# MohamedAbou-Taleb/Iterative-Linear-Quadratic-Regulator

Hardware: AMD Instinct MI355X
Metric: iLQR iterations/sec (batch=4096, T=200, n=4 m=1); backward-pass HBM GB/s (higher is better)
Workload: dtype f32; 1 GPU; c3: under-actuated double pendulum swing-up (run_iLQR_UA_MPC.py params), n=4 m=1 N=200 rk4, batch 4096 trajectories per GPU, 10 parallel line-search alphas per pass covering the 10 reference trials, fixed iterations; batch_per_gpu=4096, horizon=200, n_alpha=10, n_trials=10

## Files before the change

### iterative-linear-quadratic-regulator_amd/csrc/backward_fused16.hpp

```cpp
#pragma once

namespace ilqr {

template <typename T, int TPW, bool PK> struct FusedCfg;
template <> struct FusedCfg<float, 16, false> { static constexpr int P = 8, RU = 8; };
#ifndef ILQR_PK_RU
#define ILQR_PK_RU 5
#endif
#ifndef ILQR_PK_PAD
#define ILQR_PK_PAD 0
#endif
template <> struct FusedCfg<float, 16, true> { static constexpr int P = 4, RU = ILQR_PK_RU; };
template <> struct FusedCfg<double, 16, false> { static constexpr int P = 4, RU = 4; };
template <> struct FusedCfg<float, 4, false> { static constexpr int P = 3, RU = 4; };
template <> struct FusedCfg<double, 4, false> { static constexpr int P = 3, RU = 3; };

template <int NU> constexpr int fused_tl() { return NU == 2 ? 68 : 52; }
template <bool PK, int NU> constexpr int fused_unit_scalars() { return (PK ? 128 : 64) * fused_tl<NU>() + (PK ? 64 * ILQR_PK_PAD : 0); }
template <typename T, int TPW, bool PK, int NU> constexpr int fused_ru() { return (PK && NU == 2 && FusedCfg<T, TPW, PK>::RU > 4) ? 4 : FusedCfg<T, TPW, PK>::RU; }
template <typename T, int TPW, bool PK, int NU = 1> constexpr int fused_lds_bytes() {
    return fused_ru<T, TPW, PK, NU>() * fused_unit_scalars<PK, NU>() * (int)sizeof(T) + (fused_ru<T, TPW, PK, NU>() + 4 + 32 + 4) * 4;
}
static_assert(fused_lds_bytes<float, 16, true, 1>() <= 160 * 1024 && fused_lds_bytes<float, 16, true, 2>() <= 160 * 1024 &&
              fused_lds_bytes<float, 16, false, 2>() <= 160 * 1024 && fused_lds_bytes<double, 16, false, 2>() <= 160 * 1024, "LDS ring exceeds a CU");
template <typename T, int TPW, bool PK> constexpr int fused_threads() { return 64 * (TPW / 4 + FusedCfg<T, TPW, PK>::P); }

template <typename T, int NU> struct FusedStep;
template <> struct FusedStep<float, 1> {
    using Tile = TileQ;
    static ILQR_DEV void load(Tile& t, const float* tp, int i, int j, int l16) {
        const float4 s = *reinterpret_cast<const float4*>(tp + 4 * j);
        const float4 v = *reinterpret_cast<const float4*>(tp + 32 + 4 * j);
        t.skj[0] = s.x; t.skj[1] = s.y; t.skj[2] = s.z; t.skj[3] = s.w;
        t.vj[0] = v.x; t.vj[1] = v.y; t.vj[2] = v.z; t.vj[3] = v.w;
        t.a = tp[l16];
        t.lxx = tp[16 + l16];
        t.c = tp[32 + l16];
    }
    static ILQR_DEV void step(const Tile& c, const LaneConst<float>& lc, int i, int j, float& V, float& vx, float& out, bool& pd) {
        RawTileQ none;
        const i32x4 srd = {0, 0, 0, 0};
        const TileOffsets off = {0, 0, 0};
        float Kj, kff;
        tile16_step_f32<false>(c, lc, V, vx, Kj, kff, pd, none, srd, off, 0);
        out = (i == 0) ? Kj : kff;
    }
    static ILQR_DEV void step_box(const Tile& c, const LaneConst<float>& lc, int i, int j, float u, float lo, float hi,
                                  float& V, float& vx, float& out, bool& pd) {
        RawTileQ none;
        const i32x4 srd = {0, 0, 0, 0};
        const TileOffsets off = {0, 0, 0};
        float Kj, kff;
        tile16_step_f32<false, true>(c, lc, V, vx, Kj, kff, pd, none, srd, off, 0, u, lo, hi);
        out = (i == 0) ? Kj : kff;
    }
};
template <> struct FusedStep<double, 1> {
    using Tile = Tile16<double>;
    static ILQR_DEV void load(Tile& t, const double* tp, int i, int j, int l16) { tile16_load_lds(t, tp, i, j, l16); }
    static ILQR_DEV void step(const Tile& c, const LaneConst<double>& lc, int i, int j, double& V, double& vx, double& out, bool& pd) {
        double Kj, kff;
        tile16_step<double, false>(c, lc, 0.0, V, vx, Kj, kff, pd);
        out = (i == 0) ? Kj : kff;
    }
    static ILQR_DEV void step_box(const Tile& c, const LaneConst<double>& lc, int i, int j, double u, double lo, double hi,
                                  double& V, double& vx, double& out, bool& pd) {
        double Kj, kff;
        tile16_step<double, false, true>(c, lc, 0.0, V, vx, Kj, kff, pd, u, lo, hi);
        out = (i == 0) ? Kj : kff;
    }
};
template <> struct FusedStep<float, 2> {
    using Tile = TileQ2;
    static ILQR_DEV void load(Tile& t, const float* tp, int i, int j, int l16) { tileq2_load_lds(t, tp, i, j, l16); }
    static ILQR_DEV void step(const Tile& c, const LaneConst<float>& lc, int i, int j, float& V, float& vx, float& out, bool& pd) {
        const GainSel sel = GainSel::of(i, j);
        tile16m2_step_f32(c, lc, sel, V, vx, out, pd);
    }
};
template <typename T> struct FusedStep<T, 2> {
    using Tile = Tile16M2<T>;
    using V4 = typename Vec4<T>::type;
    static ILQR_DEV void load(Tile& t, const T* tp, int i, int j, int l16) {
        const V4 si = *reinterpret_cast<const V4*>(tp + 4 * i);
        const V4 sj = *reinterpret_cast<const V4*>(tp + 4 * j);
        const V4 g0 = *reinterpret_cast<const V4*>(tp + 32 + 8 * j);
        const V4 g1 = *reinterpret_cast<const V4*>(tp + 36 + 8 * j);
        t.ski[0] = si.x; t.ski[1] = si.y; t.ski[2] = si.z; t.ski[3] = si.w;
        t.skj[0] = sj.x; t.skj[1] = sj.y; t.skj[2] = sj.z; t.skj[3] = sj.w;
        t.gj[0] = g0.x; t.gj[1] = g0.y; t.gj[2] = g0.z; t.gj[3] = g0.w;
        t.gj[4] = g1.x; t.gj[5] = g1.y; t.gj[6] = g1.z; t.gj[7] = g1.w;
        const T* gi = tp + 32 + 8 * i;
        t.gi[0] = gi[0]; t.gi[1] = gi[1]; t.gi[3] = gi[3]; t.gi[4] = gi[4];
        t.lxx = tp[16 + l16];
    }
    static ILQR_DEV void step(const Tile& c, const LaneConst<T>& lc, int i, int j, T& V, T& vx, T& out, bool& pd) {
        T K0, K1, k0, k1;
        tile16m2_step<T, false>(c, lc.m0, lc.m1, T(0), V, vx, K0, K1, k0, k1, pd);
        out = (i == 0) ? K0 : ((i == 1) ? K1 : ((j == 0) ? k0 : k1));
    }
};

ILQR_DEV void compiler_fence() { asm volatile("" ::: "memory"); }
ILQR_DEV int lds_peek(const int* p) { return __hip_atomic_load(p, __ATOMIC_RELAXED, __HIP_MEMORY_SCOPE_WORKGROUP); }
ILQR_DEV void lds_poke(int* p, int v) { __hip_atomic_store(p, v, __ATOMIC_RELAXED, __HIP_MEMORY_SCOPE_WORKGROUP); }

template <typename T, typename Dyn, int INTEG, int TPW, bool PK, bool BOX, bool HET> struct FusedRoles {
    static constexpr int NX = Dyn::NX, NU = Dyn::NU;
    static_assert(!BOX || (NU == 1 && fused_tl<1>() > kTile16), "control limits: n_u = 1, u_t in the tile's padding");
    static_assert((NU == 1 && NX >= 2 && NX <= 4) || (NX == 4 && NU == 2), "the fused sweep serves the DPP tiles: n_u = 1, or (4, 2)");
    static_assert(TPW == 16 || TPW == 4, "16 or 4 trajectories per workgroup");
    static_assert(!PK || (sizeof(T) == 4 && TPW == 16 && INTEG != ILQR_INT_BACKWARD_EULER), "pair producers: fp32, 16-trajectory workgroups, explicit integrators");
    using Cfg = FusedCfg<T, TPW, PK>;
    static constexpr int P = Cfg::P, RU = fused_ru<T, TPW, PK, NU>(), TL = fused_tl<NU>();
    static constexpr int NV = (NU == 2 ? kTile16M2 : kTile16) / 4;
    static constexpr int NSW = TPW / 4;
    static constexpr int UT = PK ? 128 : 64;
    static constexpr int US = UT / TPW;
    static constexpr int UNIT = fused_unit_scalars<PK, NU>();
    static constexpr int PS = 2 * TL + ILQR_PK_PAD;
    static constexpr int R = gain_record(NX, NU);
    using PL = ParamLayout<Dyn::NSYS, NX, NU>;
    using V4 = typename Vec4<T>::type;
    static ILQR_DEV constexpr int tile_off(int r, int tl) { return PK ? ((r / 2) * TPW + tl) * PS + (r % 2) * TL : (r * TPW + tl) * TL; }
    static ILQR_DEV constexpr int step_off(int r) { return PK ? (r / 2) * TPW * PS + (r % 2) * TL : r * TPW * TL; }

    struct Lds {
        T* ring;
        int* ready;
        int* done;
        int* s_slot;
        int* s_stat;
    };
    static ILQR_DEV Lds carve(unsigned char* base) {
        Lds L;
        L.ring = reinterpret_cast<T*>(base);
        L.ready = reinterpret_cast<int*>(base + (size_t)RU * UNIT * sizeof(T));
        L.done = L.ready + RU;
        L.s_slot = L.done + 4;
        L.s_stat = L.s_slot + 16;
        return L;
    }

    static ILQR_DEV void head(const KArgs<T>& a, const Lds& L, int b0, int lane, bool do_select, bool count) {
        bool still = false;
        if (lane < 16) {
            const int b = b0 + lane;
            int slot = 0, st = -1;
            if (lane < TPW && b < a.B) {
                if (do_select) {
                    still = select_candidates(a, b, true, slot, st);
                } else {
                    st = a.status[b];
                    slot = a.cur_slot[b];
                }
                a.cur_slot[b] = traj_active(st) ? 0 : slot;
            }
            L.s_slot[lane] = slot;
            L.s_stat[lane] = st;
        } else if (lane < 16 + RU + 4) {
            L.ready[lane - 16] = 0;
        }
        if (do_select && count) {
            const unsigned long long m = __ballot(still);
            if (lane == 0 && m) atomicAdd(&a.counters[a.counter_idx], (int)__popcll(m));
            if (blockIdx.x == 0 && lane == 0) a.counters[(a.counter_idx + 1) % kCounterRing] = 0;
        }
    }
    static ILQR_DEV bool any_active(const Lds& L) {
        bool any = false;
#pragma unroll
        for (int q = 0; q < 16; ++q) any = any || traj_active(L.s_stat[q]);
        return any;
    }

    static ILQR_DEV void sweep(const KArgs<T>& a, const Lds& L, int b0, int wave, int lane, ClockProbe& cp) {
        const size_t B = a.B;
        const int N = a.N;
        const int tid = threadIdx.x;
        (void)tid;
        __builtin_amdgcn_s_setprio(2);
        const int l16 = lane & 15, i = l16 >> 2, j = l16 & 3;
        const int tl = 4 * wave + (lane >> 4);
        const int gidx = b0 + tl;
        const bool valid = gidx < a.B;
        const int b = valid ? gidx : a.B - 1;
        const int st = L.s_stat[tl];
        const bool act = valid && traj_active(st);
        const int slot = act ? L.s_slot[tl] : 0;
        T ph[HET ? PL::TOTAL : 1];
        if constexpr (HET) {
#pragma unroll
            for (int q = 0; q < PL::TOTAL; ++q) ph[q] = a.params[q];
            load_row<PL::Q>(ph, a.rows, B, b);
        }
        const T* __restrict__ pp = HET ? ph : a.params;
        T xN[NX];
        vec_load<T, NX>(a.X + vec_at(B, N + 1, NX, slot, N, b), xN);
        if (act && slot != 0 && l16 == 0) vec_store<T, NX>(a.X + vec_at(B, N + 1, NX, 0, N, b), xN);
        T V = T(0), vx = T(0);
        {
            T g[NX], H[NX][NX];
            Cost<T, Dyn>::l_f_x(pp, xN, g);
            Cost<T, Dyn>::l_f_xx(pp, xN, H);
#pragma unroll
            for (int ii = 0; ii < NX; ++ii) {
// ... 254 lines not shown
```

### iterative-linear-quadratic-regulator_amd/csrc/backward_tile16.hpp

```cpp
#pragma once
#include <type_traits>
#include <utility>

#include "dynamics.hpp"

namespace ilqr {

constexpr int dpp_quad(int a, int b, int c, int d) { return a | (b << 2) | (c << 4) | (d << 6); }
constexpr int kRowRor = 0x120;
constexpr int kDown1 = kRowRor + 12;
constexpr int kDown2 = kRowRor + 8;
constexpr int kDown3 = kRowRor + 4;
constexpr int kRight1 = dpp_quad(1, 2, 3, 0);
constexpr int kRight2 = dpp_quad(2, 3, 0, 1);
constexpr int kRight3 = dpp_quad(3, 0, 1, 2);
constexpr int kSwap1 = dpp_quad(1, 0, 3, 2);

template <int CTRL, int BANK = 0xf, bool BOUND = true> ILQR_DEV int dpp_bits(int old, int v) {
    return __builtin_amdgcn_update_dpp(old, v, CTRL, 0xf, BANK, BOUND);
}
template <int CTRL> ILQR_DEV float dpp(float v) {
    return __int_as_float(dpp_bits<CTRL>(0, __float_as_int(v)));
}
template <int CTRL> ILQR_DEV double dpp(double v) {
// ... 224 lines not shown
    float a, lxx, c;
    ILQR_DEV void issue_first(const i32x4& srd, const TileOffsets& o, int soff) {
        asm volatile(
            "s_nop 4\n\t"
            "buffer_load_dwordx4 %0, %5, %7, %8 offen" ILQR_TILE_NT "\n\t"
            "buffer_load_dwordx4 %1, %5, %7, %8 offen offset:128" ILQR_TILE_NT "\n\t"
            "buffer_load_dword %2, %6, %7, %8 offen" ILQR_TILE_NT "\n\t"
            "buffer_load_dword %3, %6, %7, %8 offen offset:64" ILQR_TILE_NT "\n\t"
            "buffer_load_dword %4, %6, %7, %8 offen offset:128" ILQR_TILE_NT
            : "=&v"(skj), "=&v"(vj), "=&v"(a), "=&v"(lxx), "=&v"(c)
            : "v"(o.vj), "v"(o.vl), "s"(srd), "s"(soff)
            : "memory");
    }
#define ILQR_RAWTILE_PART(NOP, dst, voff, IMM)                                                               \
    asm volatile(NOP "buffer_load_dword" IMM ILQR_TILE_NT : "+&v"(dst) : "v"(voff), "s"(srd), "s"(soff) : "memory")
    template <int K> ILQR_DEV void issue_part(const i32x4& srd, const TileOffsets& o, int soff) {
        if constexpr (K == 0) ILQR_RAWTILE_PART("s_nop 4\n\t", skj, o.vj, "x4 %0, %1, %2, %3 offen");
        if constexpr (K == 1) ILQR_RAWTILE_PART("", vj, o.vj, "x4 %0, %1, %2, %3 offen offset:128");
        if constexpr (K == 2) ILQR_RAWTILE_PART("", a, o.vl, " %0, %1, %2, %3 offen");
        if constexpr (K == 3) ILQR_RAWTILE_PART("", lxx, o.vl, " %0, %1, %2, %3 offen offset:64");
        if constexpr (K == 4) ILQR_RAWTILE_PART("", c, o.vl, " %0, %1, %2, %3 offen offset:128");
    }
    template <int N> ILQR_DEV void wait() {
        asm volatile("s_waitcnt vmcnt(%5)" : "+v"(skj), "+v"(vj), "+v"(a), "+v"(lxx), "+v"(c) : "i"(N) : "memory");
    }
    ILQR_DEV void unpack(TileQ& t) const {
        t.skj[0] = skj.x; t.skj[1] = skj.y; t.skj[2] = skj.z; t.skj[3] = skj.w;
        t.vj[0] = vj.x; t.vj[1] = vj.y; t.vj[2] = vj.z; t.vj[3] = vj.w;
        t.a = a; t.lxx = lxx; t.c = c;
    }
};

#define ILQR_FMAC_DPP_(NOP, acc, w, coef, CTRL)                                                        \
    asm volatile(NOP "v_fmac_f32_dpp %0, %1, %2 " CTRL " row_mask:0xf bank_mask:0xf bound_ctrl:1"        \
                 : "+v"(acc)                                                                           \
                 : "v"(w), "v"(coef))
#define ILQR_FMAC_DPP_FIRST(acc, w, coef, CTRL) ILQR_FMAC_DPP_("s_nop 1\n\t", acc, w, coef, CTRL)
#define ILQR_FMAC_DPP_NEXT(acc, w, coef, CTRL) ILQR_FMAC_DPP_("", acc, w, coef, CTRL)

ILQR_DEV float contract_row(const float* skj, float w, float init) {
    float acc = fmaf(skj[0], w, init);
    ILQR_FMAC_DPP_FIRST(acc, w, skj[1], "quad_perm:[1,2,3,0]");
    ILQR_FMAC_DPP_NEXT(acc, w, skj[2], "quad_perm:[2,3,0,1]");
    ILQR_FMAC_DPP_NEXT(acc, w, skj[3], "quad_perm:[3,0,1,2]");
    return acc;
}
ILQR_DEV double contract_row(const double* skj, double w, double init) {
    double acc = fma(skj[0], w, init);
    acc += skj[1] * dpp<kRight1>(w);
    acc += skj[2] * dpp<kRight2>(w);
    acc += skj[3] * dpp<kRight3>(w);
    return acc;
}
ILQR_DEV float contract_col(const float* ski, float w) {
    float acc = ski[0] * w;
    ILQR_FMAC_DPP_FIRST(acc, w, ski[1], "row_ror:12");
    ILQR_FMAC_DPP_NEXT(acc, w, ski[2], "row_ror:8");
    ILQR_FMAC_DPP_NEXT(acc, w, ski[3], "row_ror:4");
    return acc;
}
ILQR_DEV double contract_col(const double* ski, double w) {
    double acc = ski[0] * w;
    acc += ski[1] * dpp<kDown1>(w);
    acc += ski[2] * dpp<kDown2>(w);
    acc += ski[3] * dpp<kDown3>(w);
    return acc;
}
template <typename T> ILQR_DEV T quad_sum(T v) {
    v += dpp<kSwap1>(v);
    v += dpp<kRight2>(v);
    return v;
}

ILQR_DEV float lane_transpose(float v, int src_byte) {
    return __int_as_float(__builtin_amdgcn_ds_bpermute(src_byte, __float_as_int(v)));
}
ILQR_DEV double lane_transpose(double v, int src_byte) {
    const int lo = __builtin_amdgcn_ds_bpermute(src_byte, __double2loint(v));
    const int hi = __builtin_amdgcn_ds_bpermute(src_byte, __double2hiint(v));
    return __hiloint2double(hi, lo);
}

ILQR_DEV void contract_row2(const float* skj, float w0, float w1, float c0, float c1, float& o0, float& o1) {
    float a0 = fmaf(skj[0], w0, c0), a1 = fmaf(skj[0], w1, c1);
    ILQR_FMAC_DPP_FIRST(a0, w0, skj[1], "quad_perm:[1,2,3,0]");
    ILQR_FMAC_DPP_NEXT(a1, w1, skj[1], "quad_perm:[1,2,3,0]");
    ILQR_FMAC_DPP_NEXT(a0, w0, skj[2], "quad_perm:[2,3,0,1]");
    ILQR_FMAC_DPP_NEXT(a1, w1, skj[2], "quad_perm:[2,3,0,1]");
    ILQR_FMAC_DPP_NEXT(a0, w0, skj[3], "quad_perm:[3,0,1,2]");
    ILQR_FMAC_DPP_NEXT(a1, w1, skj[3], "quad_perm:[3,0,1,2]");
    o0 = a0; o1 = a1;
}
ILQR_DEV void contract_row2(const double* skj, double w0, double w1, double c0, double c1, double& o0, double& o1) {
    o0 = contract_row(skj, w0, c0);
    o1 = contract_row(skj, w1, c1);
}

template <typename T> struct LaneConst {
    T m0, m1;
    int tr_byte;
};

template <typename T, bool REG, bool BOX = false>
ILQR_DEV void tile16_step(const Tile16<T>& c, const LaneConst<T>& lc, T mu, T& V, T& vx, T& Kj, T& kff, bool& pd,
                          T ut = T(0), T blo = T(0), T bhi = T(0)) {
    static_assert(!(BOX && REG), "control limits take the fused kernels, which run without regularisation");
    const T P = contract_col(c.ski, V);
    T pu = c.bi * V;
    pu += dpp<kDown2>(pu);
    pu += dpp<kDown1>(pu);
    T Qux, Qx;
    contract_row2(c.skj, pu, vx, c.vj[2], c.vj[1], Qux, Qx);
    const T Quu = quad_sum(lc.m1 * c.vj[3] + pu * c.vj[0]);
    const T Qu = quad_sum(lc.m0 * c.vj[3] + c.vj[0] * vx);
    const T Qr = REG ? Quu + mu : Quu;
    pd = Qr > T(0);
    const T inv = fast_rcp(Qr);
    Kj = -(Qux * inv);
    kff = -(Qu * inv);
    T Quxi = Qux;
    Quxi = dpp_row<dpp_quad(0, 0, 0, 0), 0x1>(Quxi, Qux);
    Quxi = dpp_row<dpp_quad(1, 1, 1, 1), 0x2>(Quxi, Qux);
    Quxi = dpp_row<dpp_quad(2, 2, 2, 2), 0x4>(Quxi, Qux);
    Quxi = dpp_row<dpp_quad(3, 3, 3, 3), 0x8>(Quxi, Qux);
    const T Qxx = contract_row(c.skj, P, c.lxx);
    if constexpr (!REG) {
        V = Qxx + Quxi * Kj;
        vx = Qx + Kj * Qu;
        if constexpr (BOX) {
            const T lo = blo - ut, hi = bhi - ut;
            const bool out = kff < lo || kff > hi;
            const T kc = clamp_keep_nan(kff, lo, hi);
            const T vxc = Qx + Qux * kc;
            V = out ? Qxx : V;
            vx = out ? vxc : vx;
            Kj = out ? T(0) : Kj;
            kff = kc;
        }
    } else {
        const T Ki = -(Quxi * inv);
        V = Qxx + Ki * (Quu * Kj) + Ki * Qux + Quxi * Kj;
        vx = Qx + Kj * (Quu * kff + Qu) + Qux * kff;
    }
}

#define ILQR_QP1 "quad_perm:[1,2,3,0]"
#define ILQR_QP2 "quad_perm:[2,3,0,1]"
#define ILQR_QP3 "quad_perm:[3,0,1,2]"
#define ILQR_QSW "quad_perm:[1,0,3,2]"
#define ILQR_QB0 "quad_perm:[0,0,0,0]"
#define ILQR_QB1 "quad_perm:[1,1,1,1]"
#define ILQR_QB2 "quad_perm:[2,2,2,2]"
#define ILQR_QB3 "quad_perm:[3,3,3,3]"
template <bool REFILL, bool BOX = false>
ILQR_DEV void tile16_step_f32(const TileQ& c, const LaneConst<float>& lc, float& V, float& vx, float& Kj, float& kff,
                              bool& pd, RawTileQ& prev, const i32x4& srd, const TileOffsets& off, int soff,
                              float ut = 0.0f, float blo = 0.0f, float bhi = 0.0f) {
    using T = float;
    float P, pu, qx, qu, quu, Qxx, Qux, Quxi, t, t2, inv, si1, si2, si3;
#define DPPT " row_mask:0xf bank_mask:0xf bound_ctrl:1\n\t"
#define DPPE " row_mask:0xf bank_mask:0xf bound_ctrl:1"
    asm volatile(
        "v_mov_b32_dpp %[si1], %[a] " ILQR_QB1 DPPT
        "v_mov_b32_dpp %[si2], %[a] " ILQR_QB2 DPPT
        "v_mov_b32_dpp %[si3], %[a] " ILQR_QB3 DPPT
        "v_mul_f32_dpp %[P], %[a], %[V] " ILQR_QB0 DPPT
        "v_mul_f32_dpp %[pu], %[c], %[V] " ILQR_QB0 DPPT
        "v_fma_f32 %[qx], %[sj0], %[vx], %[vj1]\n\t"
        "v_fmac_f32_dpp %[P], %[V], %[si1] row_ror:12" DPPT
        "v_add_f32_dpp %[t], %[pu], %[pu] row_ror:8" DPPE
        : [P] "=&v"(P), [pu] "=&v"(pu), [qx] "=&v"(qx), [t] "=&v"(t), [si1] "=&v"(si1), [si2] "=&v"(si2), [si3] "=&v"(si3)
        : [V] "v"(V), [vx] "v"(vx), [a] "v"(c.a), [c] "v"(c.c), [sj0] "v"(c.skj[0]), [vj1] "v"(c.vj[1]));
    if constexpr (REFILL) prev.template issue_part<0>(srd, off, soff);
    asm volatile(
        "v_fmac_f32_dpp %[qx], %[vx], %[sj1] " ILQR_QP1 DPPT
        "v_fmac_f32_dpp %[P], %[V], %[si2] row_ror:8" DPPT
        "v_add_f32_dpp %[pu], %[t], %[t] row_ror:12" DPPT
        "v_mul_f32 %[qu], %[vj0], %[vx]\n\t"
        "v_fmac_f32_dpp %[qx], %[vx], %[sj2] " ILQR_QP2 DPPT
        "v_fmac_f32_dpp %[P], %[V], %[si3] row_ror:4" DPPE
        : [qx] "+v"(qx), [P] "+v"(P), [qu] "=&v"(qu), [pu] "=&v"(pu)
        : [V] "v"(V), [vx] "v"(vx), [si2] "v"(si2), [si3] "v"(si3), [sj1] "v"(c.skj[1]), [sj2] "v"(c.skj[2]),
          [vj0] "v"(c.vj[0]), [t] "v"(t));
    if constexpr (REFILL) prev.template issue_part<1>(srd, off, soff);
    asm volatile(
        "v_mul_f32 %[quu], %[pu], %[vj0]\n\t"
        "v_fma_f32 %[Qux], %[sj0], %[pu], %[vj2]\n\t"
        "v_fmac_f32_dpp %[qx], %[vx], %[sj3] " ILQR_QP3 DPPT
        "v_fmac_f32 %[quu], %[m1], %[vj3]\n\t"
        "v_fmac_f32 %[qu], %[m0], %[vj3]\n\t"
        "v_fma_f32 %[Qxx], %[sj0], %[P], %[lxx]"
        : [quu] "=&v"(quu), [Qux] "=&v"(Qux), [Qxx] "=&v"(Qxx), [qx] "+v"(qx), [qu] "+v"(qu)
        : [vx] "v"(vx), [sj0] "v"(c.skj[0]), [sj3] "v"(c.skj[3]), [vj0] "v"(c.vj[0]), [vj2] "v"(c.vj[2]),
          [vj3] "v"(c.vj[3]), [lxx] "v"(c.lxx), [m0] "v"(lc.m0), [m1] "v"(lc.m1), [pu] "v"(pu), [P] "v"(P));
    if constexpr (REFILL) prev.template issue_part<2>(srd, off, soff);
    asm volatile(
        "v_fmac_f32_dpp %[Qux], %[pu], %[sj1] " ILQR_QP1 DPPT
        "v_add_f32_dpp %[t2], %[quu], %[quu] " ILQR_QSW DPPT
        "v_add_f32_dpp %[t], %[qu], %[qu] " ILQR_QSW DPPT
        "v_fmac_f32_dpp %[Qxx], %[P], %[sj1] " ILQR_QP1 DPPT
        "v_add_f32_dpp %[quu], %[t2], %[t2] " ILQR_QP2 DPPT
        "v_fmac_f32_dpp %[Qux], %[pu], %[sj2] " ILQR_QP2 DPPE
        : [Qux] "+v"(Qux), [Qxx] "+v"(Qxx), [quu] "+v"(quu), [t] "=&v"(t), [t2] "=&v"(t2)
        : [sj1] "v"(c.skj[1]), [sj2] "v"(c.skj[2]), [pu] "v"(pu), [P] "v"(P), [qu] "v"(qu));
    if constexpr (REFILL) prev.template issue_part<3>(srd, off, soff);
    asm volatile(
        "v_add_f32_dpp %[qu], %[t], %[t] " ILQR_QP2 DPPT
        "v_rcp_f32 %[inv], %[quu]\n\t"
        "v_fmac_f32_dpp %[Qxx], %[P], %[sj2] " ILQR_QP2 DPPT
        "v_fmac_f32_dpp %[Qux], %[pu], %[sj3] " ILQR_QP3 DPPT
        "v_fma_f32 %[e], -%[quu], %[inv], 1.0\n\t"
        "v_fmac_f32_dpp %[Qxx], %[P], %[sj3] " ILQR_QP3 DPPT
        "v_mov_b32_dpp %[Quxi], %[Qux] " ILQR_QB0 " row_mask:0xf bank_mask:0x1\n\t"
        "v_fmac_f32 %[inv], %[e], %[inv]\n\t"
        "v_mov_b32_dpp %[Quxi], %[Qux] " ILQR_QB1 " row_mask:0xf bank_mask:0x2\n\t"
        "v_mov_b32_dpp %[Quxi], %[Qux] " ILQR_QB2 " row_mask:0xf bank_mask:0x4\n\t"
        "v_mov_b32_dpp %[Quxi], %[Qux] " ILQR_QB3 " row_mask:0xf bank_mask:0x8"
        : [Quxi] "=&v"(Quxi), [Qxx] "+v"(Qxx), [Qux] "+v"(Qux), [qu] "=&v"(qu), [inv] "=&v"(inv), [e] "=&v"(t2)
        : [sj2] "v"(c.skj[2]), [sj3] "v"(c.skj[3]), [pu] "v"(pu), [P] "v"(P), [t] "v"(t), [quu] "v"(quu));
    if constexpr (REFILL) prev.template issue_part<4>(srd, off, soff);
#undef DPPT
#undef DPPE
    pd = quu > 0.0f;
    Kj = -(Qux * inv);
    kff = -(qu * inv);
    V = fmaf(Quxi, Kj, Qxx);
    vx = fmaf(Kj, qu, qx);
    if constexpr (BOX) {
        const T lo = blo - ut, hi = bhi - ut;
        const bool out = kff < lo || kff > hi;
        const T kc = clamp_keep_nan(kff, lo, hi);
        const T vxc = fmaf(Qux, kc, qx);
        V = out ? Qxx : V;
        vx = out ? vxc : vx;
        Kj = out ? T(0) : Kj;
        kff = kc;
    }
}

constexpr int kTile16PinLds = 84 * 1024;

template <typename T, bool REG, int NXA>
__global__ void __launch_bounds__(256) backward_tile16_kernel(KArgs<T> a) {
#ifndef ILQR_TILE16_D32
#define ILQR_TILE16_D32 10
#endif
    constexpr bool SPREAD = sizeof(T) == 4 && !REG;
    constexpr int D = SPREAD ? ILQR_TILE16_D32 : sizeof(T) == 4 ? 10 : 7;
    constexpr int R = gain_record(NXA, 1);
    const int lane = threadIdx.x & 63;
    const int l16 = lane & 15, i = l16 >> 2, j = l16 & 3;
    const int gidx = (blockIdx.x * 4 + (threadIdx.x >> 6)) * 4 + (lane >> 4);
    const bool valid = gidx < a.B;
    const int b = valid ? gidx : a.B - 1;
    const int st = a.status[b];
    const bool act = valid && traj_active(st);
    if (__ballot(act) == 0ull) return;
    if (a.reset_slots && act && l16 == 0) a.cur_slot[b] = 0;
    ClockProbe cp;
    cp.start();
    const size_t B = a.B;
    const int N = a.N;
    T V = a.term[(size_t)(4 + l16) * B + b];
    T vx = a.term[(size_t)j * B + b];
    const unsigned lin_bytes = (unsigned)((size_t)N * B * kTile16 * sizeof(T));
    const unsigned gain_bytes = (unsigned)((size_t)N * B * R * sizeof(T));
    const __amdgpu_buffer_rsrc_t rlin = make_rsrc(a.lin, lin_bytes);
    const __amdgpu_buffer_rsrc_t rgain = make_rsrc(a.gains, gain_bytes);
    const int tstride = (int)(B * kTile16 * sizeof(T));
    const int rstride = (int)(B * R * sizeof(T));
    TileOffsets off;
    off.vi = (int)((b * kTile16 + 4 * i) * sizeof(T));
    off.vj = (int)((b * kTile16 + 4 * j) * sizeof(T));
    off.vl = (int)((b * kTile16 + l16) * sizeof(T));
    constexpr bool DROP = sizeof(T) == 4 || ILQR_DROP_ALL;
    const bool storer = act && ((i == 0 && j < NXA) || l16 == 4);
    const int rec_off = (storer || !DROP) ? (int)((b * R + (i == 0 ? j : NXA)) * sizeof(T)) : 0x7ffffff0;
    bool all_pd = true;
    LaneConst<T> lc;
    lc.m0 = T(j == 0);
    lc.m1 = T(j == 1);
    lc.tr_byte = 4 * ((lane & 48) | (j << 2) | i);

    int t = N - 1;
    if constexpr (SPREAD) {
        const i32x4 srd = make_srd(a.lin, lin_bytes);
        int goff = t * rstride, roff = 0;
        auto step = [&](auto refill, const TileQ& c, RawTileQ& prev) {
            T Kj, kff;
            bool pd;
#ifdef ILQR_T16_NOLOAD
            tile16_step_f32<false>(c, lc, V, vx, Kj, kff, pd, prev, srd, off, uniform(roff > 0 ? roff : 0));
#else
            tile16_step_f32<decltype(refill)::value>(c, lc, V, vx, Kj, kff, pd, prev, srd, off,
                                                     uniform(roff > 0 ? roff : 0));
#endif
            all_pd = all_pd && pd;
#ifndef ILQR_T16_NOSTORE
            buf_store1(rgain, rec_off, uniform(goff), (i == 0) ? Kj : kff);
#else
            if (a.N == 123457) buf_store1(rgain, rec_off, uniform(goff), (i == 0) ? Kj : kff);
#endif
            goff -= rstride;
            roff -= tstride;
        };
        RawTileQ ring[D];
#ifdef ILQR_T16_STAMPS
        long long stamp_cal = 0, stamp_wait = 0;
        const long long stamp_t0 = __builtin_readcyclecounter();
#endif
        for (int r = N % D; r > 0; --r, --t) {
            TileQ c;
            tileq_load_buf(c, rlin, off, uniform(t * tstride));
            step(std::false_type{}, c, ring[0]);
        }
        if (t >= 0) {
            constexpr int NL = RawTileQ::NLOAD;
#pragma unroll
            for (int u = 0; u < D; ++u) ring[u].issue_first(srd, off, uniform((t - u) * tstride));
            static_assert(1 + (D - 2) * (NL + 1) <= 63 && (D - 1) * NL <= 63, "vmcnt field");
            roff = (t + 1 - D) * tstride;
            static_for<D>([&](auto uc) {
                constexpr int u = decltype(uc)::value;
                ring[u].template wait<(u == 0) ? (D - 1) * NL : (D - 2) * NL + u>();
                TileQ c;
                ring[u].unpack(c);
                if constexpr (u == 0) step(std::false_type{}, c, ring[0]);
                else step(std::true_type{}, c, ring[u - 1]);
            });
            for (t -= D; t >= 0; t -= D) {
                static_for<D>([&](auto uc) {
                    constexpr int u = decltype(uc)::value;
#ifdef ILQR_T16_STAMPS
                    const long long w0 = __builtin_readcyclecounter();
                    const long long w1 = __builtin_readcyclecounter();
                    ring[u].template wait<1 + (D - 2) * (NL + 1)>();
                    const long long w2 = __builtin_readcyclecounter();
                    stamp_cal += w1 - w0;
                    stamp_wait += w2 - w1;
#else
                    ring[u].template wait<1 + (D - 2) * (NL + 1)>();
#endif
                    TileQ c;
                    ring[u].unpack(c);
                    step(std::true_type{}, c, ring[(u + D - 1) % D]);
                });
            }
            asm volatile("s_waitcnt vmcnt(0)" ::: "memory");
        }
#ifdef ILQR_T16_STAMPS
        if (a.probe && blockIdx.x == 7 && threadIdx.x == 0) {
            a.probe[2] = stamp_wait; a.probe[3] = stamp_cal; a.probe[4] = __builtin_readcyclecounter() - stamp_t0;
        }
#endif
    } else {
        auto do_step = [&](const Tile16<T>& c, int t) {
            T Kj, kff;
            bool pd;
            tile16_step<T, REG>(c, lc, a.mu, V, vx, Kj, kff, pd);
            all_pd = all_pd && pd;
            if (DROP || storer) buf_store1(rgain, rec_off, uniform(t * rstride), (i == 0) ? Kj : kff);
        };
        for (int r = N % D; r > 0; --r, --t) {
            Tile16<T> c;
            tile16_load_buf(c, rlin, off, uniform(t * tstride));
            do_step(c, t);
        }
        if (t >= 0) {
            constexpr int NL = RawTile<T>::NLOAD;
            const i32x4 srd = make_srd(a.lin, lin_bytes);
            RawTile<T> ring[D];
#pragma unroll
            for (int u = 0; u < D; ++u) ring[u].template issue<true>(srd, off, uniform((t - u) * tstride));
// ... 183 lines not shown
```

### iterative-linear-quadratic-regulator_amd/csrc/fwd_in_gen.inc

```
template <typename T, int NX, int NU> struct FwdIn;
template <> struct FwdIn<float, 2, 1> {
    static constexpr int R = 4, GV = 1, NLD = 3;
    typedef unsigned int u4 __attribute__((ext_vector_type(4)));
    typedef unsigned int u2 __attribute__((ext_vector_type(2)));
    u2 xp[1];
    unsigned int up[1];
    u4 g[1];
#define ILQR_FWDIN_ASM(OUT) \
        asm volatile( \
            "s_nop 4\n\t" \
            "buffer_load_dwordx2 %0, %3, %6, %9 offen\n\t" \
            "buffer_load_dword %1, %4, %7, %10 offen\n\t" \
            "buffer_load_dwordx4 %2, %5, %8, %11 offen" \
            : OUT(xp[0]), OUT(up[0]), OUT(g[0]) \
            : "v"(vx), "v"(vu), "v"(vg), "s"(srdX), "s"(srdU), "s"(srdG), "s"(sxu), "s"(suu), "s"(sgu) \
            : "memory")
    template <bool FIRST>
    ILQR_DEV void issue(__amdgpu_buffer_rsrc_t srdX, __amdgpu_buffer_rsrc_t srdU, __amdgpu_buffer_rsrc_t srdG, int vx, int vu, int vg, int sx,
                        int su, int sg) {
        const int sxu = uniform(sx), suu = uniform(su), sgu = uniform(sg);
        if constexpr (FIRST) ILQR_FWDIN_ASM(ILQR_OUT_FIRST);
        else ILQR_FWDIN_ASM(ILQR_OUT_REFILL);
    }
#undef ILQR_FWDIN_ASM
    template <int N> ILQR_DEV void wait() {
        asm volatile("s_waitcnt vmcnt(%3)" : "+v"(xp[0]), "+v"(up[0]), "+v"(g[0]) : "i"(N) : "memory");
    }
    ILQR_DEV void unpack(float* xo, float* uo) const {
        xo[0] = __uint_as_float(xp[0][0]);
        xo[1] = __uint_as_float(xp[0][1]);
        uo[0] = __uint_as_float(up[0]);
    }
    ILQR_DEV float gain(int r) const {
        return __uint_as_float(g[r / 4][r % 4]);
    }
};
template <> struct FwdIn<float, 4, 1> {
    static constexpr int R = 8, GV = 2, NLD = 4;
    typedef unsigned int u4 __attribute__((ext_vector_type(4)));
    typedef unsigned int u2 __attribute__((ext_vector_type(2)));
    u4 xp[1];
    unsigned int up[1];
    u4 g[2];
#define ILQR_FWDIN_ASM(OUT) \
        asm volatile( \
            "s_nop 4\n\t" \
            "buffer_load_dwordx4 %0, %4, %7, %10 offen\n\t" \
            "buffer_load_dword %1, %5, %8, %11 offen\n\t" \
            "buffer_load_dwordx4 %2, %6, %9, %12 offen\n\t" \
            "buffer_load_dwordx4 %3, %6, %9, %12 offen offset:16" \
            : OUT(xp[0]), OUT(up[0]), OUT(g[0]), OUT(g[1]) \
            : "v"(vx), "v"(vu), "v"(vg), "s"(srdX), "s"(srdU), "s"(srdG), "s"(sxu), "s"(suu), "s"(sgu) \
            : "memory")
    template <bool FIRST>
    ILQR_DEV void issue(__amdgpu_buffer_rsrc_t srdX, __amdgpu_buffer_rsrc_t srdU, __amdgpu_buffer_rsrc_t srdG, int vx, int vu, int vg, int sx,
                        int su, int sg) {
        const int sxu = uniform(sx), suu = uniform(su), sgu = uniform(sg);
        if constexpr (FIRST) ILQR_FWDIN_ASM(ILQR_OUT_FIRST);
        else ILQR_FWDIN_ASM(ILQR_OUT_REFILL);
    }
#undef ILQR_FWDIN_ASM
    template <int N> ILQR_DEV void wait() {
        asm volatile("s_waitcnt vmcnt(%4)" : "+v"(xp[0]), "+v"(up[0]), "+v"(g[0]), "+v"(g[1]) : "i"(N) : "memory");
    }
    ILQR_DEV void unpack(float* xo, float* uo) const {
        xo[0] = __uint_as_float(xp[0][0]);
        xo[1] = __uint_as_float(xp[0][1]);
        xo[2] = __uint_as_float(xp[0][2]);
        xo[3] = __uint_as_float(xp[0][3]);
        uo[0] = __uint_as_float(up[0]);
    }
    ILQR_DEV float gain(int r) const {
        return __uint_as_float(g[r / 4][r % 4]);
    }
};
template <> struct FwdIn<float, 4, 2> {
    static constexpr int R = 12, GV = 3, NLD = 5;
    typedef unsigned int u4 __attribute__((ext_vector_type(4)));
    typedef unsigned int u2 __attribute__((ext_vector_type(2)));
    u4 xp[1];
    u2 up[1];
    u4 g[3];
#define ILQR_FWDIN_ASM(OUT) \
        asm volatile( \
            "s_nop 4\n\t" \
            "buffer_load_dwordx4 %0, %5, %8, %11 offen\n\t" \
            "buffer_load_dwordx2 %1, %6, %9, %12 offen\n\t" \
            "buffer_load_dwordx4 %2, %7, %10, %13 offen\n\t" \
            "buffer_load_dwordx4 %3, %7, %10, %13 offen offset:16\n\t" \
            "buffer_load_dwordx4 %4, %7, %10, %13 offen offset:32" \
            : OUT(xp[0]), OUT(up[0]), OUT(g[0]), OUT(g[1]), OUT(g[2]) \
            : "v"(vx), "v"(vu), "v"(vg), "s"(srdX), "s"(srdU), "s"(srdG), "s"(sxu), "s"(suu), "s"(sgu) \
            : "memory")
    template <bool FIRST>
    ILQR_DEV void issue(__amdgpu_buffer_rsrc_t srdX, __amdgpu_buffer_rsrc_t srdU, __amdgpu_buffer_rsrc_t srdG, int vx, int vu, int vg, int sx,
                        int su, int sg) {
        const int sxu = uniform(sx), suu = uniform(su), sgu = uniform(sg);
        if constexpr (FIRST) ILQR_FWDIN_ASM(ILQR_OUT_FIRST);
        else ILQR_FWDIN_ASM(ILQR_OUT_REFILL);
    }
#undef ILQR_FWDIN_ASM
    template <int N> ILQR_DEV void wait() {
        asm volatile("s_waitcnt vmcnt(%5)" : "+v"(xp[0]), "+v"(up[0]), "+v"(g[0]), "+v"(g[1]), "+v"(g[2]) : "i"(N) : "memory");
    }
    ILQR_DEV void unpack(float* xo, float* uo) const {
        xo[0] = __uint_as_float(xp[0][0]);
        xo[1] = __uint_as_float(xp[0][1]);
        xo[2] = __uint_as_float(xp[0][2]);
        xo[3] = __uint_as_float(xp[0][3]);
        uo[0] = __uint_as_float(up[0][0]);
        uo[1] = __uint_as_float(up[0][1]);
    }
    ILQR_DEV float gain(int r) const {
        return __uint_as_float(g[r / 4][r % 4]);
    }
};
template <> struct FwdIn<double, 2, 1> {
    static constexpr int R = 4, GV = 2, NLD = 4;
    typedef unsigned int u4 __attribute__((ext_vector_type(4)));
    typedef unsigned int u2 __attribute__((ext_vector_type(2)));
    u4 xp[1];
    u2 up[1];
    u4 g[2];
#define ILQR_FWDIN_ASM(OUT) \
        asm volatile( \
            "s_nop 4\n\t" \
            "buffer_load_dwordx4 %0, %4, %7, %10 offen\n\t" \
            "buffer_load_dwordx2 %1, %5, %8, %11 offen\n\t" \
            "buffer_load_dwordx4 %2, %6, %9, %12 offen\n\t" \
            "buffer_load_dwordx4 %3, %6, %9, %12 offen offset:16" \
            : OUT(xp[0]), OUT(up[0]), OUT(g[0]), OUT(g[1]) \
            : "v"(vx), "v"(vu), "v"(vg), "s"(srdX), "s"(srdU), "s"(srdG), "s"(sxu), "s"(suu), "s"(sgu) \
            : "memory")
    template <bool FIRST>
    ILQR_DEV void issue(__amdgpu_buffer_rsrc_t srdX, __amdgpu_buffer_rsrc_t srdU, __amdgpu_buffer_rsrc_t srdG, int vx, int vu, int vg, int sx,
                        int su, int sg) {
        const int sxu = uniform(sx), suu = uniform(su), sgu = uniform(sg);
        if constexpr (FIRST) ILQR_FWDIN_ASM(ILQR_OUT_FIRST);
        else ILQR_FWDIN_ASM(ILQR_OUT_REFILL);
    }
#undef ILQR_FWDIN_ASM
    template <int N> ILQR_DEV void wait() {
        asm volatile("s_waitcnt vmcnt(%4)" : "+v"(xp[0]), "+v"(up[0]), "+v"(g[0]), "+v"(g[1]) : "i"(N) : "memory");
    }
    ILQR_DEV void unpack(double* xo, double* uo) const {
        xo[0] = __hiloint2double((int)xp[0][1], (int)xp[0][0]);
        xo[1] = __hiloint2double((int)xp[0][3], (int)xp[0][2]);
        uo[0] = __hiloint2double((int)up[0][1], (int)up[0][0]);
    }
    ILQR_DEV double gain(int r) const {
        return __hiloint2double((int)g[r / 2][2 * (r % 2) + 1], (int)g[r / 2][2 * (r % 2)]);
    }
};
template <> struct FwdIn<double, 4, 1> {
    static constexpr int R = 8, GV = 4, NLD = 7;
    typedef unsigned int u4 __attribute__((ext_vector_type(4)));
    typedef unsigned int u2 __attribute__((ext_vector_type(2)));
    u4 xp[2];
    u2 up[1];
    u4 g[4];
#define ILQR_FWDIN_ASM(OUT) \
        asm volatile( \
            "s_nop 4\n\t" \
            "buffer_load_dwordx4 %0, %7, %10, %13 offen\n\t" \
            "buffer_load_dwordx4 %1, %7, %10, %13 offen offset:16\n\t" \
            "buffer_load_dwordx2 %2, %8, %11, %14 offen\n\t" \
            "buffer_load_dwordx4 %3, %9, %12, %15 offen\n\t" \
            "buffer_load_dwordx4 %4, %9, %12, %15 offen offset:16\n\t" \
            "buffer_load_dwordx4 %5, %9, %12, %15 offen offset:32\n\t" \
            "buffer_load_dwordx4 %6, %9, %12, %15 offen offset:48" \
            : OUT(xp[0]), OUT(xp[1]), OUT(up[0]), OUT(g[0]), OUT(g[1]), OUT(g[2]), OUT(g[3]) \
            : "v"(vx), "v"(vu), "v"(vg), "s"(srdX), "s"(srdU), "s"(srdG), "s"(sxu), "s"(suu), "s"(sgu) \
            : "memory")
    template <bool FIRST>
    ILQR_DEV void issue(__amdgpu_buffer_rsrc_t srdX, __amdgpu_buffer_rsrc_t srdU, __amdgpu_buffer_rsrc_t srdG, int vx, int vu, int vg, int sx,
                        int su, int sg) {
        const int sxu = uniform(sx), suu = uniform(su), sgu = uniform(sg);
        if constexpr (FIRST) ILQR_FWDIN_ASM(ILQR_OUT_FIRST);
        else ILQR_FWDIN_ASM(ILQR_OUT_REFILL);
    }
#undef ILQR_FWDIN_ASM
    template <int N> ILQR_DEV void wait() {
        asm volatile("s_waitcnt vmcnt(%7)" : "+v"(xp[0]), "+v"(xp[1]), "+v"(up[0]), "+v"(g[0]), "+v"(g[1]), "+v"(g[2]), "+v"(g[3]) : "i"(N) : "memory");
    }
    ILQR_DEV void unpack(double* xo, double* uo) const {
        xo[0] = __hiloint2double((int)xp[0][1], (int)xp[0][0]);
        xo[1] = __hiloint2double((int)xp[0][3], (int)xp[0][2]);
        xo[2] = __hiloint2double((int)xp[1][1], (int)xp[1][0]);
        xo[3] = __hiloint2double((int)xp[1][3], (int)xp[1][2]);
        uo[0] = __hiloint2double((int)up[0][1], (int)up[0][0]);
    }
    ILQR_DEV double gain(int r) const {
        return __hiloint2double((int)g[r / 2][2 * (r % 2) + 1], (int)g[r / 2][2 * (r % 2)]);
    }
};
template <> struct FwdIn<double, 4, 2> {
    static constexpr int R = 12, GV = 6, NLD = 9;
    typedef unsigned int u4 __attribute__((ext_vector_type(4)));
    typedef unsigned int u2 __attribute__((ext_vector_type(2)));
    u4 xp[2];
    u4 up[1];
    u4 g[6];
#define ILQR_FWDIN_ASM(OUT) \
        asm volatile( \
            "s_nop 4\n\t" \
            "buffer_load_dwordx4 %0, %9, %12, %15 offen\n\t" \
            "buffer_load_dwordx4 %1, %9, %12, %15 offen offset:16\n\t" \
            "buffer_load_dwordx4 %2, %10, %13, %16 offen\n\t" \
            "buffer_load_dwordx4 %3, %11, %14, %17 offen\n\t" \
            "buffer_load_dwordx4 %4, %11, %14, %17 offen offset:16\n\t" \
            "buffer_load_dwordx4 %5, %11, %14, %17 offen offset:32\n\t" \
            "buffer_load_dwordx4 %6, %11, %14, %17 offen offset:48\n\t" \
            "buffer_load_dwordx4 %7, %11, %14, %17 offen offset:64\n\t" \
            "buffer_load_dwordx4 %8, %11, %14, %17 offen offset:80" \
            : OUT(xp[0]), OUT(xp[1]), OUT(up[0]), OUT(g[0]), OUT(g[1]), OUT(g[2]), OUT(g[3]), OUT(g[4]), OUT(g[5]) \
            : "v"(vx), "v"(vu), "v"(vg), "s"(srdX), "s"(srdU), "s"(srdG), "s"(sxu), "s"(suu), "s"(sgu) \
            : "memory")
    template <bool FIRST>
    ILQR_DEV void issue(__amdgpu_buffer_rsrc_t srdX, __amdgpu_buffer_rsrc_t srdU, __amdgpu_buffer_rsrc_t srdG, int vx, int vu, int vg, int sx,
                        int su, int sg) {
        const int sxu = uniform(sx), suu = uniform(su), sgu = uniform(sg);
        if constexpr (FIRST) ILQR_FWDIN_ASM(ILQR_OUT_FIRST);
        else ILQR_FWDIN_ASM(ILQR_OUT_REFILL);
    }
#undef ILQR_FWDIN_ASM
    template <int N> ILQR_DEV void wait() {
        asm volatile("s_waitcnt vmcnt(%9)" : "+v"(xp[0]), "+v"(xp[1]), "+v"(up[0]), "+v"(g[0]), "+v"(g[1]), "+v"(g[2]), "+v"(g[3]), "+v"(g[4]), "+v"(g[5]) : "i"(N) : "memory");
    }
    ILQR_DEV void unpack(double* xo, double* uo) const {
        xo[0] = __hiloint2double((int)xp[0][1], (int)xp[0][0]);
        xo[1] = __hiloint2double((int)xp[0][3], (int)xp[0][2]);
        xo[2] = __hiloint2double((int)xp[1][1], (int)xp[1][0]);
        xo[3] = __hiloint2double((int)xp[1][3], (int)xp[1][2]);
        uo[0] = __hiloint2double((int)up[0][1], (int)up[0][0]);
        uo[1] = __hiloint2double((int)up[0][3], (int)up[0][2]);
    }
    ILQR_DEV double gain(int r) const {
        return __hiloint2double((int)g[r / 2][2 * (r % 2) + 1], (int)g[r / 2][2 * (r % 2)]);
    }
};
```

Measured before the change: 29.63 million iLQR iterations/sec.

## Use full-row LDS tile view in fused f32 step and trim forward gain loads

The fused float backward step now loads a full Tile16 from LDS (ski row values and bi per lane) instead of the compact TileQ. A new FULL variant of the f32 step drops the DPP broadcasts that rebuilt those row values, shortening the dependency chain at the cost of more registers and LDS reads. The forward-input loaders for the 4x1 and 4x2 cases also stop fetching padding dwords of the gain rows, loading only the needed gain words with a narrower last load.

```diff
diff --git a/iterative-linear-quadratic-regulator_amd/csrc/backward_fused16.hpp b/iterative-linear-quadratic-regulator_amd/csrc/backward_fused16.hpp
--- a/iterative-linear-quadratic-regulator_amd/csrc/backward_fused16.hpp
+++ b/iterative-linear-quadratic-regulator_amd/csrc/backward_fused16.hpp
@@ -27,22 +27,14 @@
 
 template <typename T, int NU> struct FusedStep;
 template <> struct FusedStep<float, 1> {
-    using Tile = TileQ;
-    static ILQR_DEV void load(Tile& t, const float* tp, int i, int j, int l16) {
-        const float4 s = *reinterpret_cast<const float4*>(tp + 4 * j);
-        const float4 v = *reinterpret_cast<const float4*>(tp + 32 + 4 * j);
-        t.skj[0] = s.x; t.skj[1] = s.y; t.skj[2] = s.z; t.skj[3] = s.w;
-        t.vj[0] = v.x; t.vj[1] = v.y; t.vj[2] = v.z; t.vj[3] = v.w;
-        t.a = tp[l16];
-        t.lxx = tp[16 + l16];
-        t.c = tp[32 + l16];
-    }
+    using Tile = Tile16<float>;
+    static ILQR_DEV void load(Tile& t, const float* tp, int i, int j, int l16) { tile16_load_lds(t, tp, i, j, l16); }
     static ILQR_DEV void step(const Tile& c, const LaneConst<float>& lc, int i, int j, float& V, float& vx, float& out, bool& pd) {
         RawTileQ none;
         const i32x4 srd = {0, 0, 0, 0};
         const TileOffsets off = {0, 0, 0};
         float Kj, kff;
-        tile16_step_f32<false>(c, lc, V, vx, Kj, kff, pd, none, srd, off, 0);
+        tile16_step_f32<false, false, true>(c, lc, V, vx, Kj, kff, pd, none, srd, off, 0);
         out = (i == 0) ? Kj : kff;
     }
     static ILQR_DEV void step_box(const Tile& c, const LaneConst<float>& lc, int i, int j, float u, float lo, float hi,
@@ -51,7 +43,7 @@
         const i32x4 srd = {0, 0, 0, 0};
         const TileOffsets off = {0, 0, 0};
         float Kj, kff;
-        tile16_step_f32<false, true>(c, lc, V, vx, Kj, kff, pd, none, srd, off, 0, u, lo, hi);
+        tile16_step_f32<false, true, true>(c, lc, V, vx, Kj, kff, pd, none, srd, off, 0, u, lo, hi);
         out = (i == 0) ? Kj : kff;
     }
 };
diff --git a/iterative-linear-quadratic-regulator_amd/csrc/backward_tile16.hpp b/iterative-linear-quadratic-regulator_amd/csrc/backward_tile16.hpp
--- a/iterative-linear-quadratic-regulator_amd/csrc/backward_tile16.hpp
+++ b/iterative-linear-quadratic-regulator_amd/csrc/backward_tile16.hpp
@@ -400,14 +400,59 @@
 #define ILQR_QB1 "quad_perm:[1,1,1,1]"
 #define ILQR_QB2 "quad_perm:[2,2,2,2]"
 #define ILQR_QB3 "quad_perm:[3,3,3,3]"
-template <bool REFILL, bool BOX = false>
-ILQR_DEV void tile16_step_f32(const TileQ& c, const LaneConst<float>& lc, float& V, float& vx, float& Kj, float& kff,
-                              bool& pd, RawTileQ& prev, const i32x4& srd, const TileOffsets& off, int soff,
-                              float ut = 0.0f, float blo = 0.0f, float bhi = 0.0f) {
+template <bool REFILL, bool BOX = false, bool FULL = false>
+ILQR_DEV void tile16_step_f32(const std::conditional_t<FULL, Tile16<float>, TileQ>& c, const LaneConst<float>& lc, float& V,
+                              float& vx, float& Kj, float& kff, bool& pd, RawTileQ& prev, const i32x4& srd,
+                              const TileOffsets& off, int soff, float ut = 0.0f, float blo = 0.0f, float bhi = 0.0f) {
+    static_assert(!(FULL && REFILL), "the full-row view is read from LDS: there is no ring refill to spread");
     using T = float;
     float P, pu, qx, qu, quu, Qxx, Qux, Quxi, t, t2, inv, si1, si2, si3;
 #define DPPT " row_mask:0xf bank_mask:0xf bound_ctrl:1\n\t"
 #define DPPE " row_mask:0xf bank_mask:0xf bound_ctrl:1"
+    if constexpr (FULL) {
+    (void)si1; (void)si2; (void)si3;
+    asm volatile(
+        "v_mul_f32 %[P], %[si0], %[V]\n\t"
+        "v_mul_f32 %[pu], %[bi], %[V]\n\t"
+        "v_fma_f32 %[qx], %[sj0], %[vx], %[vj1]\n\t"
+        "v_fmac_f32_dpp %[P], %[V], %[si1] row_ror:12" DPPT
+        "v_add_f32_dpp %[t], %[pu], %[pu] row_ror:8" DPPT
+        "v_fmac_f32_dpp %[qx], %[vx], %[sj1] " ILQR_QP1 DPPT
+        "v_fmac_f32_dpp %[P], %[V], %[si2] row_ror:8" DPPT
+        "v_add_f32_dpp %[pu], %[t], %[t] row_ror:12" DPPT
+        "v_mul_f32 %[qu], %[vj0], %[vx]\n\t"
+        "v_fmac_f32_dpp %[qx], %[vx], %[sj2] " ILQR_QP2 DPPT
+        "v_fmac_f32_dpp %[P], %[V], %[si3] row_ror:4" DPPT
+        "v_mul_f32 %[quu], %[pu], %[vj0]\n\t"
+        "v_fma_f32 %[Qux], %[sj0], %[pu], %[vj2]\n\t"
+        "v_fmac_f32_dpp %[qx], %[vx], %[sj3] " ILQR_QP3 DPPT
+        "v_fmac_f32 %[quu], %[m1], %[vj3]\n\t"
+        "v_fmac_f32 %[qu], %[m0], %[vj3]\n\t"
+        "v_fma_f32 %[Qxx], %[sj0], %[P], %[lxx]\n\t"
+        "v_fmac_f32_dpp %[Qux], %[pu], %[sj1] " ILQR_QP1 DPPT
+        "v_add_f32_dpp %[e], %[quu], %[quu] " ILQR_QSW DPPT
+        "v_add_f32_dpp %[t], %[qu], %[qu] " ILQR_QSW DPPT
+        "v_fmac_f32_dpp %[Qxx], %[P], %[sj1] " ILQR_QP1 DPPT
+        "v_add_f32_dpp %[quu], %[e], %[e] " ILQR_QP2 DPPT
+        "v_fmac_f32_dpp %[Qux], %[pu], %[sj2] " ILQR_QP2 DPPT
+        "v_add_f32_dpp %[qu], %[t], %[t] " ILQR_QP2 DPPT
+        "v_rcp_f32 %[inv], %[quu]\n\t"
+        "v_fmac_f32_dpp %[Qxx], %[P], %[sj2] " ILQR_QP2 DPPT
+        "v_fmac_f32_dpp %[Qux], %[pu], %[sj3] " ILQR_QP3 DPPT
+        "v_fma_f32 %[e], -%[quu], %[inv], 1.0\n\t"
+        "v_fmac_f32_dpp %[Qxx], %[P], %[sj3] " ILQR_QP3 DPPT
+        "v_mov_b32_dpp %[Quxi], %[Qux] " ILQR_QB0 " row_mask:0xf bank_mask:0x1\n\t"
+        "v_fmac_f32 %[inv], %[e], %[inv]\n\t"
+        "v_mov_b32_dpp %[Quxi], %[Qux] " ILQR_QB1 " row_mask:0xf bank_mask:0x2\n\t"
+        "v_mov_b32_dpp %[Quxi], %[Qux] " ILQR_QB2 " row_mask:0xf bank_mask:0x4\n\t"
+        "v_mov_b32_dpp %[Quxi], %[Qux] " ILQR_QB3 " row_mask:0xf bank_mask:0x8"
+        : [P] "=&v"(P), [pu] "=&v"(pu), [qx] "=&v"(qx), [t] "=&v"(t), [qu] "=&v"(qu), [quu] "=&v"(quu), [Qux] "=&v"(Qux),
+          [Qxx] "=&v"(Qxx), [e] "=&v"(t2), [Quxi] "=&v"(Quxi), [inv] "=&v"(inv)
+        : [V] "v"(V), [vx] "v"(vx), [si0] "v"(c.ski[0]), [si1] "v"(c.ski[1]), [si2] "v"(c.ski[2]), [si3] "v"(c.ski[3]),
+          [bi] "v"(c.bi), [sj0] "v"(c.skj[0]), [sj1] "v"(c.skj[1]), [sj2] "v"(c.skj[2]), [sj3] "v"(c.skj[3]),
+          [vj0] "v"(c.vj[0]), [vj1] "v"(c.vj[1]), [vj2] "v"(c.vj[2]), [vj3] "v"(c.vj[3]), [lxx] "v"(c.lxx),
+          [m0] "v"(lc.m0), [m1] "v"(lc.m1));
+    } else {
     asm volatile(
         "v_mov_b32_dpp %[si1], %[a] " ILQR_QB1 DPPT
         "v_mov_b32_dpp %[si2], %[a] " ILQR_QB2 DPPT
@@ -467,6 +512,7 @@
         : [Quxi] "=&v"(Quxi), [Qxx] "+v"(Qxx), [Qux] "+v"(Qux), [qu] "=&v"(qu), [inv] "=&v"(inv), [e] "=&v"(t2)
         : [sj2] "v"(c.skj[2]), [sj3] "v"(c.skj[3]), [pu] "v"(pu), [P] "v"(P), [t] "v"(t), [quu] "v"(quu));
     if constexpr (REFILL) prev.template issue_part<4>(srd, off, soff);
+    }
 #undef DPPT
 #undef DPPE
     pd = quu > 0.0f;
diff --git a/iterative-linear-quadratic-regulator_amd/csrc/fwd_in_gen.inc b/iterative-linear-quadratic-regulator_amd/csrc/fwd_in_gen.inc
--- a/iterative-linear-quadratic-regulator_amd/csrc/fwd_in_gen.inc
+++ b/iterative-linear-quadratic-regulator_amd/csrc/fwd_in_gen.inc
@@ -41,27 +41,28 @@
     typedef unsigned int u2 __attribute__((ext_vector_type(2)));
     u4 xp[1];
     unsigned int up[1];
-    u4 g[2];
+    u4 g[1];
+    unsigned int g1;
 #define ILQR_FWDIN_ASM(OUT) \
         asm volatile( \
             "s_nop 4\n\t" \
             "buffer_load_dwordx4 %0, %4, %7, %10 offen\n\t" \
             "buffer_load_dword %1, %5, %8, %11 offen\n\t" \
             "buffer_load_dwordx4 %2, %6, %9, %12 offen\n\t" \
-            "buffer_load_dwordx4 %3, %6, %9, %12 offen offset:16" \
-            : OUT(xp[0]), OUT(up[0]), OUT(g[0]), OUT(g[1]) \
-            : "v"(vx), "v"(vu), "v"(vg), "s"(srdX), "s"(srdU), "s"(srdG), "s"(sxu), "s"(suu), "s"(sgu) \
-            : "memory")
-    template <bool FIRST>
-    ILQR_DEV void issue(__amdgpu_buffer_rsrc_t srdX, __amdgpu_buffer_rsrc_t srdU, __amdgpu_buffer_rsrc_t srdG, int vx, int vu, int vg, int sx,
-                        int su, int sg) {
-        const int sxu = uniform(sx), suu = uniform(su), sgu = uniform(sg);
-        if constexpr (FIRST) ILQR_FWDIN_ASM(ILQR_OUT_FIRST);
-        else ILQR_FWDIN_ASM(ILQR_OUT_REFILL);
-    }
-#undef ILQR_FWDIN_ASM
-    template <int N> ILQR_DEV void wait() {
-        asm volatile("s_waitcnt vmcnt(%4)" : "+v"(xp[0]), "+v"(up[0]), "+v"(g[0]), "+v"(g[1]) : "i"(N) : "memory");
+            "buffer_load_dword %3, %6, %9, %12 offen offset:16" \
+            : OUT(xp[0]), OUT(up[0]), OUT(g[0]), OUT(g1) \
+            : "v"(vx), "v"(vu), "v"(vg), "s"(srdX), "s"(srdU), "s"(srdG), "s"(sxu), "s"(suu), "s"(sgu) \
+            : "memory")
+    template <bool FIRST>
+    ILQR_DEV void issue(__amdgpu_buffer_rsrc_t srdX, __amdgpu_buffer_rsrc_t srdU, __amdgpu_buffer_rsrc_t srdG, int vx, int vu, int vg, int sx,
+                        int su, int sg) {
+        const int sxu = uniform(sx), suu = uniform(su), sgu = uniform(sg);
+        if constexpr (FIRST) ILQR_FWDIN_ASM(ILQR_OUT_FIRST);
+        else ILQR_FWDIN_ASM(ILQR_OUT_REFILL);
+    }
+#undef ILQR_FWDIN_ASM
+    template <int N> ILQR_DEV void wait() {
+        asm volatile("s_waitcnt vmcnt(%4)" : "+v"(xp[0]), "+v"(up[0]), "+v"(g[0]), "+v"(g1) : "i"(N) : "memory");
     }
     ILQR_DEV void unpack(float* xo, float* uo) const {
         xo[0] = __uint_as_float(xp[0][0]);
@@ -71,7 +72,11 @@
         uo[0] = __uint_as_float(up[0]);
     }
     ILQR_DEV float gain(int r) const {
-        return __uint_as_float(g[r / 4][r % 4]);
+        if (r == 0) return __uint_as_float(g[0][0]);
+        if (r == 1) return __uint_as_float(g[0][1]);
+        if (r == 2) return __uint_as_float(g[0][2]);
+        if (r == 3) return __uint_as_float(g[0][3]);
+        return __uint_as_float(g1);
     }
 };
 template <> struct FwdIn<float, 4, 2> {
@@ -80,7 +85,8 @@
     typedef unsigned int u2 __attribute__((ext_vector_type(2)));
     u4 xp[1];
     u2 up[1];
-    u4 g[3];
+    u4 g[2];
+    u2 g2;
 #define ILQR_FWDIN_ASM(OUT) \
         asm volatile( \
             "s_nop 4\n\t" \
@@ -88,20 +94,20 @@
             "buffer_load_dwordx2 %1, %6, %9, %12 offen\n\t" \
             "buffer_load_dwordx4 %2, %7, %10, %13 offen\n\t" \
             "buffer_load_dwordx4 %3, %7, %10, %13 offen offset:16\n\t" \
-            "buffer_load_dwordx4 %4, %7, %10, %13 offen offset:32" \
-            : OUT(xp[0]), OUT(up[0]), OUT(g[0]), OUT(g[1]), OUT(g[2]) \
-            : "v"(vx), "v"(vu), "v"(vg), "s"(srdX), "s"(srdU), "s"(srdG), "s"(sxu), "s"(suu), "s"(sgu) \
-            : "memory")
-    template <bool FIRST>
-    ILQR_DEV void issue(__amdgpu_buffer_rsrc_t srdX, __amdgpu_buffer_rsrc_t srdU, __amdgpu_buffer_rsrc_t srdG, int vx, int vu, int vg, int sx,
-                        int su, int sg) {
-        const int sxu = uniform(sx), suu = uniform(su), sgu = uniform(sg);
-        if constexpr (FIRST) ILQR_FWDIN_ASM(ILQR_OUT_FIRST);
-        else ILQR_FWDIN_ASM(ILQR_OUT_REFILL);
-    }
-#undef ILQR_FWDIN_ASM
-    template <int N> ILQR_DEV void wait() {
-        asm volatile("s_waitcnt vmcnt(%5)" : "+v"(xp[0]), "+v"(up[0]), "+v"(g[0]), "+v"(g[1]), "+v"(g[2]) : "i"(N) : "memory");
+            "buffer_load_dwordx2 %4, %7, %10, %13 offen offset:32" \
+            : OUT(xp[0]), OUT(up[0]), OUT(g[0]), OUT(g[1]), OUT(g2) \
+            : "v"(vx), "v"(vu), "v"(vg), "s"(srdX), "s"(srdU), "s"(srdG), "s"(sxu), "s"(suu), "s"(sgu) \
+            : "memory")
+    template <bool FIRST>
+    ILQR_DEV void issue(__amdgpu_buffer_rsrc_t srdX, __amdgpu_buffer_rsrc_t srdU, __amdgpu_buffer_rsrc_t srdG, int vx, int vu, int vg, int sx,
+                        int su, int sg) {
+        const int sxu = uniform(sx), suu = uniform(su), sgu = uniform(sg);
+        if constexpr (FIRST) ILQR_FWDIN_ASM(ILQR_OUT_FIRST);
+        else ILQR_FWDIN_ASM(ILQR_OUT_REFILL);
+    }
+#undef ILQR_FWDIN_ASM
+    template <int N> ILQR_DEV void wait() {
+        asm volatile("s_waitcnt vmcnt(%5)" : "+v"(xp[0]), "+v"(up[0]), "+v"(g[0]), "+v"(g[1]), "+v"(g2) : "i"(N) : "memory");
     }
     ILQR_DEV void unpack(float* xo, float* uo) const {
         xo[0] = __uint_as_float(xp[0][0]);
@@ -112,7 +118,16 @@
         uo[1] = __uint_as_float(up[0][1]);
     }
     ILQR_DEV float gain(int r) const {
-        return __uint_as_float(g[r / 4][r % 4]);
+        if (r == 0) return __uint_as_float(g[0][0]);
+        if (r == 1) return __uint_as_float(g[0][1]);
+        if (r == 2) return __uint_as_float(g[0][2]);
+        if (r == 3) return __uint_as_float(g[0][3]);
+        if (r == 4) return __uint_as_float(g[1][0]);
+        if (r == 5) return __uint_as_float(g[1][1]);
+        if (r == 6) return __uint_as_float(g[1][2]);
+        if (r == 7) return __uint_as_float(g[1][3]);
+        if (r == 8) return __uint_as_float(g2[0]);
+        return __uint_as_float(g2[1]);
     }
 };
 template <> struct FwdIn<double, 2, 1> {
```

New measurement: 29.52 million iLQR iterations/sec. Within noise of the previous version (-0.4%).
